# angelvillar96/STLPose

Measured on AMD Instinct MI355X. Metric: images/sec/GPU HRNet-W32 384x288 train step; PCKh@0.5 parity, higher is better.
Workload: dtype f16/bf16; 1 GPU; HRNet-W32 384x288 bs=32/GPU train step (fwd+MSE+bwd+Adam), random-init weights; global_batch=32, parallelism=dp1

## Files before the change

stlpose_amd/csrc/common.cuh:

```cuda
#pragma once
#include <hip/hip_runtime.h>
#include <stdint.h>
#include <stdio.h>
#include <initializer_list>
#include <tuple>
#include <type_traits>
#include <utility>
#include "../../include/stlpose_hip.h"
#include "../../include/stlpose_hip_math.h"

typedef __attribute__((ext_vector_type(4))) float f32x4;
typedef __attribute__((ext_vector_type(8))) __bf16 bf16x8;
typedef __attribute__((ext_vector_type(8))) _Float16 f16x8;
typedef __attribute__((ext_vector_type(4))) short s16x4;
struct f32s { float v; };
typedef _Float16 f16;

struct alignas(16) V16 {
    uint32_t w[4];
};

int stl_set_error(const char* fmt, ...);
void stl_note_kernel(const char* name, bool specific);
#define STL_CHECK(cond, ...)                 \
// ... 283 lines not shown
    } else {
#pragma unroll
        for (int k = 0; k < STL_NSHARD; ++k) {
            r.rs[2 * k] = s.rstats[(size_t)k * 2 * C + c];
            r.rs[2 * k + 1] = s.rstats[(size_t)k * 2 * C + C + c];
        }
    }
}
__device__ __forceinline__ void src_raw_finish(const stl_src& s, const SrcRaw& r, float& ca, float& cb, float& cc) {
#pragma clang fp contract(off)
    if (s.mode == STL_SRC_PLAIN) {
        ca = 1.f, cb = 0.f, cc = 0.f;
        return;
    }
    float mean, rstd;
    bn_raw_finish(s, r, mean, rstd);
    if (s.mode == STL_SRC_BN || s.mode == STL_SRC_BNADD) {
        ca = r.g * rstd;
        cb = fmaf(-mean, ca, r.b);
        cc = 0.f;
    } else {
        double r1 = 0.0, r2 = 0.0;
#pragma unroll
        for (int k = 0; k < STL_NSHARD; ++k) r1 += r.rs[2 * k], r2 += r.rs[2 * k + 1];
        const float c1 = (float)(r1 * (double)s.inv_count);
        const float c2 = (float)(r2 * (double)s.inv_count);
        const float al = r.g * rstd;
        ca = al;
        cb = -al * rstd * c2;
        cc = al * fmaf(mean * rstd, c2, -c1);
    }
}

__device__ __forceinline__ float row16_sum(float v) {
    v += __int_as_float(__builtin_amdgcn_update_dpp(0, __float_as_int(v), 0xB1, 0xf, 0xf, true));
    v += __int_as_float(__builtin_amdgcn_update_dpp(0, __float_as_int(v), 0x4E, 0xf, 0xf, true));
    v += __int_as_float(__builtin_amdgcn_update_dpp(0, __float_as_int(v), 0x141, 0xf, 0xf, true));
    v += __int_as_float(__builtin_amdgcn_update_dpp(0, __float_as_int(v), 0x140, 0xf, 0xf, true));
    return v;
}

__device__ __forceinline__ float wave_sum(float v) {
#pragma unroll
    for (int o = 32; o > 0; o >>= 1) v += __shfl_xor(v, o);
    return v;
}
__device__ __forceinline__ double wave_sum_d(double v) {
#pragma unroll
    for (int o = 32; o > 0; o >>= 1) v += __shfl_xor(v, o);
    return v;
}

__device__ __forceinline__ bool better(float v, int i, float bv, int bi) {
    const bool vn = v != v, bn = bv != bv;
    if (vn != bn) return vn;
    if (vn) return i < bi;
    return v > bv || (v == bv && i < bi);
}
__device__ __forceinline__ void argmax_take(float v, int i, float& bv, int& bi) {
    if (bi == 0x7fffffff || better(v, i, bv, bi)) bv = v, bi = i;
}
__device__ __forceinline__ void block_argmax_reduce(float& bv, int& bi, float* sv, int* si) {
    for (int o = 32; o > 0; o >>= 1) {
        const float ov = __shfl_xor(bv, o);
        const int oi = __shfl_xor(bi, o);
        if (oi != 0x7fffffff && (bi == 0x7fffffff || better(ov, oi, bv, bi))) bv = ov, bi = oi;
// ... 41 lines not shown
```

stlpose_amd/csrc/conv1x1.inc:

```
template <typename T, int G, bool Q, int OCC, typename TY = T, int EO = -1, bool ZM = false>
__global__ __launch_bounds__(512, OCC) void conv1x1_kernel(const ConvK k) {
    extern __shared__ __attribute__((aligned(16))) char smem[];
    constexpr int NTHR = 512, WM = 4, MT = 4, NTW = 2, BCO = 64, TPX = 256;
    constexpr int KV = ET<T>::KV, CK = ET<T>::CK;
    constexpr int PSG = G * 64 + 32;
    constexpr int VPP = 4 * G;
    constexpr int RPT = NTHR / VPP;
    constexpr int NVA = TPX / RPT;
    constexpr int NVB = BCO / RPT;
    constexpr int GK = G * CK;
    static_assert(NVB >= 1, "filter staging needs at least one vector per thread");
    const stl_conv& p = k.p;
    const int tid = threadIdx.x, lane = tid & 63, wave = tid >> 6, r16 = lane & 15, g = lane >> 4;
    const int wm = wave % WM, wn = wave / WM;
    const int bl = blockIdx.x >> 3;
    const int by = bl % k.ny, lx = bl / k.ny;
    const int n0 = by * BCO;
    const int xcd = blockIdx.x & 7, nx = (gridDim.x >> 3) / k.ny;
    const int P = p.B * p.Ho * p.Wo;

    float* cs = reinterpret_cast<float*>(smem + k.off_cs);
    float* cm = reinterpret_cast<float*>(smem + k.off_cm);
    char* sA = smem + k.off_a;
    char* sB = smem + k.off_b;

    for (int c = tid; c < k.cipad; c += NTHR) {
        float a = 0.f, b = 0.f, cc = 0.f;
        if (c < p.Ci) src_consts(p.src, c, p.Ci, a, b, cc);
        cs[c] = a, cs[k.cipad + c] = b, cs[2 * k.cipad + c] = cc;
    }
    if (p.mask_y) {
        for (int c = tid; c < BCO; c += NTHR) {
            float a = 0.f, b = 0.f, mu = 0.f, rs = 0.f;
            if (n0 + c < p.Co) {
                bn_mean_rstd(p.mask_bn, n0 + c, p.Co, mu, rs);
                bn_affine(p.mask_bn.gamma[n0 + c], p.mask_bn.beta[n0 + c], mu, rs, a, b);
            }
            cm[c] = a, cm[BCO + c] = b, cm[2 * BCO + c] = mu, cm[3 * BCO + c] = rs;
        }
    }

    const int a_part = tid % VPP, a_row = tid / VPP;
    V16 ra[NVA], rq[Q ? NVA : 1], rb[NVB];

    auto issue = [&](int P0, int k0, bool en) {
        const int ch = k0 + a_part * KV;
        const bool chok = en && ch < p.Ci;
#pragma unroll
        for (int i = 0; i < NVA; ++i) {
            const int pix = P0 + a_row + i * RPT;
            const size_t off = (chok && pix < P) ? (size_t)pix * p.Ci + ch : 0;
            ra[i] = ldg16((const char*)p.src.x + off * sizeof(T));
            if (Q) rq[i] = ldg16((const char*)p.src.y + off * sizeof(T));
        }
        if (!k.wres) {
#pragma unroll
            for (int i = 0; i < NVB; ++i) {
                const int n = n0 + a_row + i * RPT;
                const size_t off = (chok && n < p.Co) ? (size_t)n * p.Ci + ch : 0;
                rb[i] = ldg16((const char*)p.w + off * sizeof(T));
            }
        }
    };
    const float relu_lo = p.src.relu ? 0.f : -INFINITY;
    auto write_lds = [&](int P0, int k0) {
        const int ch = k0 + a_part * KV;
        const bool chok = ch < p.Ci;
        const int chc = chok ? ch : 0;
#pragma unroll
        for (int i = 0; i < NVA; ++i) {
            const bool ok = chok && (P0 + a_row + i * RPT) < P;
            V16 val = ra[i];
            if constexpr (ZM) {
                val = xform_bnadd<T>(val, rq[i], cs + chc, cs + k.cipad + chc, relu_lo);
                if (ok && by == 0 && p.src_out) stg16((char*)p.src_out + ((size_t)(P0 + a_row + i * RPT) * p.Ci + ch) * sizeof(T), val);
            } else if (Q)
                val = xform_bnbwd<T, TY>(val, rq[i], cs + chc, cs + k.cipad + chc, cs + 2 * k.cipad + chc);
            else if (p.src.mode != STL_SRC_PLAIN)
                val = xform_bn<T>(val, cs + chc, cs + k.cipad + chc, relu_lo);
            mask16(val, ok);
            *reinterpret_cast<V16*>(sA + (a_row + i * RPT) * PSG + a_part * 16) = val;
        }
        if (!k.wres) {
#pragma unroll
            for (int i = 0; i < NVB; ++i) {
                V16 val = rb[i];
                mask16(val, chok && (n0 + a_row + i * RPT) < p.Co);
                *reinterpret_cast<V16*>(sB + (a_row + i * RPT) * PSG + a_part * 16) = val;
            }
        }
    };

    if (k.wres) {
        const bool chok = a_part * KV < p.Ci;
#pragma unroll
        for (int i = 0; i < NVB; ++i) {
            const int n = n0 + a_row + i * RPT;
            const size_t off = (chok && n < p.Co) ? (size_t)n * p.Ci + a_part * KV : 0;
            rb[i] = ldg16((const char*)p.w + off * sizeof(T));
        }
    }

    f2v s0[NTW][2], s1[NTW][2];
#pragma unroll
    for (int ni = 0; ni < NTW; ++ni)
#pragma unroll
        for (int h = 0; h < 2; ++h) s0[ni][h] = f2v{0.f, 0.f}, s1[ni][h] = f2v{0.f, 0.f};
    f32x4 acc[MT][NTW];
#pragma unroll
    for (int mi = 0; mi < MT; ++mi)
#pragma unroll
        for (int ni = 0; ni < NTW; ++ni) acc[mi][ni] = f32x4{0.f, 0.f, 0.f, 0.f};

    int xoff[MT];
#pragma unroll
    for (int mi = 0; mi < MT; ++mi) xoff[mi] = ((wm * MT + mi) * 16 + r16) * PSG + g * 16;
    const int woff = (wn * NTW * 16 + r16) * PSG + g * 16;

    const int T8 = (k.npt + 7) >> 3;
    int it = lx, t = xcd * T8 + it, ch0 = 0;
    bool have = (it < T8) && (t < k.npt);
    issue(t * TPX, 0, have);
    if (k.wres) {
        const bool chok = a_part * KV < p.Ci;
#pragma unroll
        for (int i = 0; i < NVB; ++i) {
            V16 val = rb[i];
            mask16(val, chok && (n0 + a_row + i * RPT) < p.Co);
            *reinterpret_cast<V16*>(sB + (a_row + i * RPT) * PSG + a_part * 16) = val;
        }
    }
    __syncthreads();

    while (have) {
        const int P0 = t * TPX;
        write_lds(P0, ch0 * GK);
        __syncthreads();
        const bool last_chunk = (ch0 + 1 == k.nchunks);
        int itn = it, tn = t, chn = ch0 + 1;
        bool have_n = true;
        if (last_chunk) {
            itn = it + nx, tn = xcd * T8 + itn, chn = 0;
            have_n = (itn < T8) && (tn < k.npt);
        }
        issue(tn * TPX, chn * GK, have_n);
#pragma unroll
        for (int sub = 0; sub < G; ++sub) {
            V16 wf[NTW], xf[MT];
#pragma unroll
            for (int ni = 0; ni < NTW; ++ni) wf[ni] = *reinterpret_cast<const V16*>(sB + woff + ni * 16 * PSG + sub * 64);
#pragma unroll
            for (int mi = 0; mi < MT; ++mi) xf[mi] = *reinterpret_cast<const V16*>(sA + xoff[mi] + sub * 64);
#pragma unroll
            for (int mi = 0; mi < MT; ++mi)
#pragma unroll
// ... 114 lines not shown
```

stlpose_amd/csrc/conv_core.hip:

```cpp
#include <stdlib.h>
#include <algorithm>
#include <cstring>
#include <type_traits>
#include "common.cuh"

#ifndef STL_DT
#define STL_DT 2
#endif
#define STL_HAS_F32 (STL_DT == 0 || STL_DT == 2)
#define STL_HAS_BF16 (STL_DT == 1 || STL_DT == 2)
#define STL_HAS_F16 (STL_DT == 3 || STL_DT == 2)
#define STL_HAS_F32S (STL_DT == 4 || STL_DT == 2)

struct ConvK {
    stl_conv p;
    int tiles_c, npt;
    int HR, HC, HP;
    int PI, pad, seff;
    int nchunks, wres;
    int cipad;
    int off_cs, off_cm, off_a, off_b, off_red;
    int sz_a, sz_b;
    int TH, TW;
    int dbg;
// ... 48 lines not shown

#ifndef STL_PIN_TAPS
#define STL_PIN_TAPS 1
#endif
#include "conv_common.inc"

template <typename T, int KS, int WM, int WN, int MT, int NTW, int NVA, bool Q, bool PE, int OCC, int WR, bool ZM = false, typename TY = T, bool DB = false, int EO = -1>
__global__ __launch_bounds__(64 * WM * WN, OCC) void conv_core_kernel(const ConvK k) {
    extern __shared__ __attribute__((aligned(16))) char smem[];
    constexpr int NTHR = 64 * WM * WN;
    constexpr int KV = ET<T>::KV, CK = ET<T>::CK, TAPS = KS * KS;
    static_assert(!ZM || (Q && KS == 3), "block-end source: 3x3, two tensors on load");
    static_assert(!DB || (!ZM && WR == 0 && KS == 3), "double-buffered image: 3x3, plain / BN / BNBWD sources, filters staged per chunk");
    constexpr int BCO = WN * NTW * 16;
    constexpr int ROWB = TAPS * 64 + 32;
    constexpr int NVB = (BCO * TAPS * 4 + NTHR - 1) / NTHR;
    const stl_conv& p = k.p;
    const int tid = threadIdx.x, lane = tid & 63, wave = tid >> 6, r16 = lane & 15, g = lane >> 4;
    const int wm = wave % WM, wn = wave / WM;
    const int bl = blockIdx.x >> 3;
    const int lx = __builtin_amdgcn_readfirstlane(bl / k.ny), by = bl - lx * k.ny;
    const int n0 = by * BCO;
    const bool wres = WR < 0 ? (k.wres != 0) : (WR == 1);

    STAMP(0);
#ifdef STL_STAMPS
    if (k.dbg && blockIdx.x == 0 && blockIdx.y == 0 && threadIdx.x == 0) g_stamps[12] = __builtin_amdgcn_s_memtime();
#endif
    float* cs = reinterpret_cast<float*>(smem + k.off_cs);
    float* cm = reinterpret_cast<float*>(smem + k.off_cm);
    char* sA = smem + k.off_a;
    char* sB = smem + k.off_b;

    for (int c = tid; c < k.cipad; c += NTHR) {
        float a = 0.f, b = 0.f, cc = 0.f;
        if (c < p.Ci) src_consts(p.src, c, p.Ci, a, b, cc);
        cs[c] = a, cs[k.cipad + c] = b, cs[2 * k.cipad + c] = cc;
    }
    if (!PE && EpiOps<EO>::my(p)) {
        for (int c = tid - (NTHR - 64); c >= 0 && c < BCO; c += 64) {
            float a = 0.f, b = 0.f, mu = 0.f, rs = 0.f;
            if (n0 + c < p.Co) {
                bn_mean_rstd(p.mask_bn, n0 + c, p.Co, mu, rs);
                bn_affine(p.mask_bn.gamma[n0 + c], p.mask_bn.beta[n0 + c], mu, rs, a, b);
            }
            cm[c] = a, cm[BCO + c] = b, cm[2 * BCO + c] = mu, cm[3 * BCO + c] = rs;
        }
    }
    STAMP(1);
    int a_rc[NVA];
#pragma unroll
    for (int i = 0; i < NVA; ++i) {
        const int v = tid + i * NTHR;
        if (v < k.HP * 4) {
            const int hp = v >> 2, hr = fdiv(hp, k.r_HC);
            a_rc[i] = (hr << 16) | (hp - hr * k.HC);
        } else {
            a_rc[i] = -1;
        }
    }
    const int a_part = tid & 3;
    uint32_t a_int = 0;
    if constexpr (ZM) {
#pragma unroll
        for (int i = 0; i < NVA; ++i)
            if (a_rc[i] >= 0) {
                const int hr = a_rc[i] >> 16, hc = a_rc[i] & 0xffff;
                if (hr >= 1 && hr <= k.TH && hc >= 1 && hc <= k.TW && by == 0 && p.src_out) a_int |= 1u << i;
            }
    }
    int b_g[NVB], b_l[NVB];
#pragma unroll
    for (int i = 0; i < NVB; ++i) {
        const int v = tid + i * NTHR;
        b_g[i] = -1, b_l[i] = 0;
        if (v < BCO * TAPS * 4) {
            const int n = v / (TAPS * 4), r = v - n * (TAPS * 4), tap = r >> 2, part = r & 3;
            b_l[i] = n * ROWB + tap * 64 + part * 16;
            if (n0 + n < p.Co) b_g[i] = ((n0 + n) * TAPS + tap) * p.Ci + part * KV;
        }
    }
    const int tilepx = k.TH * k.TW;
    int xoff[MT];
    int e_yx[MT];
#pragma unroll
    for (int mi = 0; mi < MT; ++mi) {
        int m = (wm * MT + mi) * 16 + r16;
        e_yx[mi] = -1;
        if (m < tilepx) {
            const int ty = fdiv(m, k.r_TW);
            e_yx[mi] = (ty << 16) | (m - ty * k.TW);
        } else {
            m = 0;
        }
        const int ty = fdiv(m, k.r_TW), tx = m - ty * k.TW;
        xoff[mi] = ((ty * k.seff) * k.HC + tx * k.seff) * PSA + g * 16;
    }
    const int woff = (wn * NTW * 16 + r16) * ROWB + g * 16;

    STAMP(2);
    V16 ra[NVA], rq[Q ? NVA : 1], rb[NVB];
    int a_go[NVA];
    int st_t, st_ch;
    bool st_have;

    auto tile_terms = [&](int t, int& y0, int& cb, int& b0) __attribute__((always_inline)) {
        const int tr = sdiv(t, k.m_tc), tc = t - tr * k.tiles_c;
        const int vrs = tr * k.TH * k.seff;
        cb = tc * k.TW * k.seff - k.pad;
        b0 = sdiv(vrs, k.m_PI), y0 = vrs - b0 * k.PI - k.pad;
    };
    auto slot_go = [&](int rc, int y0, int cb, int b0) __attribute__((always_inline)) -> int {
// ... 34 lines not shown
        }
    };
    const float relu_lo = p.src.relu ? 0.f : -INFINITY;
    auto write_lds = [&](const int* go, int k0) __attribute__((always_inline)) {
        const int ch = k0 + a_part * KV;
#pragma unroll
        for (int i = 0; i < NVA; ++i) {
            if (a_rc[i] < 0) continue;
            const bool ok = go[i] >= 0 && ch < p.Ci;
            const int chc = ok ? ch : 0;
            V16 val = ra[i];
            if constexpr (ZM) {
                val = xform_bnadd<T>(val, rq[i], cs + chc, cs + k.cipad + chc, relu_lo);
                if (ok && ((a_int >> i) & 1u)) stg16((char*)p.src_out + (size_t)(go[i] + k0) * sizeof(T), val);
            } else if (Q)
                val = xform_bnbwd<T, TY>(val, rq[i], cs + chc, cs + k.cipad + chc, cs + 2 * k.cipad + chc);
            else if (p.src.mode != STL_SRC_PLAIN)
                val = xform_bn<T>(val, cs + chc, cs + k.cipad + chc, relu_lo);
            mask16(val, ok);
            const int v = tid + i * NTHR;
            *reinterpret_cast<V16*>(sA + (v >> 2) * PSA + (v & 3) * 16) = val;
        }
        if (!wres) {
#pragma unroll
            for (int i = 0; i < NVB; ++i) {
                const bool ok = b_g[i] >= 0 && (k0 + ((tid + i * NTHR) & 3) * KV) < p.Ci;
                V16 val = rb[i];
                mask16(val, ok);
                if (tid + i * NTHR < BCO * TAPS * 4) *reinterpret_cast<V16*>(sB + b_l[i]) = val;
            }
        }
    };

    if (wres) {
#pragma unroll
        for (int i = 0; i < NVB; ++i) {
            const bool ok = b_g[i] >= 0 && (((tid + i * NTHR) & 3) * KV) < p.Ci;
            rb[i] = ldg16((const char*)p.w + (size_t)(ok ? b_g[i] : 0) * sizeof(T));
        }
    }

    f2v s0[NTW][2], s1[NTW][2];
#pragma unroll
    for (int ni = 0; ni < NTW; ++ni)
#pragma unroll
        for (int h = 0; h < 2; ++h) s0[ni][h] = f2v{0.f, 0.f}, s1[ni][h] = f2v{0.f, 0.f};

    const int xcd = blockIdx.x & 7, nx = __builtin_amdgcn_readfirstlane((gridDim.x >> 3) / k.ny);
    const int T8 = (k.npt + 7) >> 3;
    const int vpitch = p.Ho + 1;

    int it_n = lx, t_n = xcd * T8 + lx, ch_n = 0;
    bool have_n = (it_n < T8) && (t_n < k.npt);
    auto prefetch = [&]() __attribute__((always_inline)) {
        if (have_n && ch_n == 0) tile_setup(t_n, a_go);
        st_t = t_n, st_ch = ch_n, st_have = have_n;
        issue(a_go, ch_n * CK, have_n);
        if (++ch_n == k.nchunks) {
            ch_n = 0, it_n += nx, t_n = xcd * T8 + it_n;
            have_n = have_n && (it_n < T8) && (t_n < k.npt);
        }
    };
    STAMP(3);
    if constexpr (!DB) {
        prefetch();
        if (wres) {
#pragma unroll
            for (int i = 0; i < NVB; ++i) {
                const bool ok = b_g[i] >= 0 && (((tid + i * NTHR) & 3) * KV) < p.Ci;
                V16 val = rb[i];
                mask16(val, ok);
                if (tid + i * NTHR < BCO * TAPS * 4) *reinterpret_cast<V16*>(sB + b_l[i]) = val;
            }
        }
        __syncthreads();
    }
    STAMP(4);

    f32x4 acc[MT][NTW];
#pragma unroll
    for (int mi = 0; mi < MT; ++mi)
#pragma unroll
        for (int ni = 0; ni < NTW; ++ni) acc[mi][ni] = f32x4{0.f, 0.f, 0.f, 0.f};

    constexpr bool EPRE = (OCC <= 1 && WM == 4 && WN == 2 && NTW == 2) && Q && !PE && !ZM && sizeof(T) == 2;
    constexpr bool EBURST = !EPRE && (EO == 1 || EO == 2) && !PE && sizeof(T) == 2;
    auto out_pixel = [&](int vr0, int c0, int mi, bool& pok) __attribute__((always_inline)) -> size_t {
        const int eb0 = sdiv(vr0, k.m_vp), ey0 = vr0 - eb0 * vpitch;
        int eyx = e_yx[mi];
        if constexpr (DB) {
            const int m = (wm * MT + mi) * 16 + r16, ty_ = fdiv(m, k.r_TW);
            eyx = m < tilepx ? ((ty_ << 16) | (m - ty_ * k.TW)) : -1;
        }
        const int ty = eyx >> 16, tx = eyx & 0xffff;
        const int oy0 = ey0 + ty, c = c0 + tx;
        const int wr_ = fdiv(oy0, k.r_vp);
        const int oy = mad24_vsv(wr_, -vpitch, oy0), b = eb0 + wr_;
        pok = (eyx >= 0) & (b < p.B) & (oy < p.Ho) & (c < p.Wo);
        const int e = mulu24_vs(madu24_vsv(madu24_vsv(b, p.Ho, oy), p.Wo, c), p.Co);
        return pok ? (size_t)(uint32_t)e : 0;
    };
    auto epi_fetch = [&](int vr0, int c0, bool* pokv, size_t* pixv, EpiRaw<NTW>* er) __attribute__((always_inline)) {
#pragma unroll
        for (int mi = 0; mi < MT; ++mi) {
            pixv[mi] = out_pixel(vr0, c0, mi, pokv[mi]);
            epilogue_fetch<T, NTW, true, EO>(p, pokv[mi], pixv[mi], n0, wn * NTW * 16, g, er[mi]);
        }
    };

    if constexpr (DB) {
        constexpr int NSLOT = NVA + NVB;
        prefetch();
        int cu_t = st_t, cu_ch = st_ch;
        bool cu_have = st_have;
        __syncthreads();
        write_lds(a_go, st_ch * CK);
        prefetch();
        __syncthreads();
        int img = 0;
        [[maybe_unused]] int dbg_it = 0;
        while (cu_have) {
            STAMP2(4 * dbg_it);
            const int t = cu_t, ch0 = cu_ch;
            const int tr = sdiv(t, k.m_tc), tc = t - tr * k.tiles_c;
            const int vr0 = tr * k.TH, c0 = tc * k.TW;
            const bool last_chunk = (ch0 + 1 == k.nchunks);
            bool pokv[EPRE ? MT : 1];
            size_t pixv[EPRE ? MT : 1];
            EpiRaw<NTW> er[EPRE ? MT : 1];
            const int k0w = st_ch * CK, k0n = ch_n * CK;
            const bool en_n = have_n, nt = have_n && ch_n == 0;
            int y0n = 0, cbn = 0, b0n = 0;
            if (nt) tile_terms(t_n, y0n, cbn, b0n);
            constexpr bool KREG = !Q || EO == 0 || EO == 1 || EO == 2;
            constexpr int NPK = sizeof(T) == 2 ? 4 : 2;
            f2v kca[NPK], kcb[NPK], kcc[Q ? NPK : 1];
            if constexpr (KREG) {
                const int ch = k0w + a_part * KV;
#pragma unroll
                for (int i = 0; i < NPK; ++i) {
                    kca[i] = reinterpret_cast<const f2v*>(cs + ch)[i];
                    kcb[i] = reinterpret_cast<const f2v*>(cs + k.cipad + ch)[i];
                    if (Q) kcc[i] = reinterpret_cast<const f2v*>(cs + 2 * k.cipad + ch)[i];
                }
            }
// ... 621 lines not shown
```

stlpose_amd/csrc/elementwise.hip:

```cpp
#include "common.cuh"

namespace {

template <typename T>
__device__ __forceinline__ void load8(const void* base, size_t elem, float* f) {
    if constexpr (sizeof(T) == 2) {
        unpack<T>(ldg16((const char*)base + elem * 2), f);
    } else {
        unpack<float>(ldg16((const char*)base + elem * 4), f);
        unpack<float>(ldg16((const char*)base + elem * 4 + 16), f + 4);
    }
}
template <typename T>
__device__ __forceinline__ void store8(void* base, size_t elem, const float* f) {
    if constexpr (sizeof(T) == 2) {
        stg16((char*)base + elem * 2, pack<T>(f));
    } else {
        stg16((char*)base + elem * 4, pack<float>(f));
        stg16((char*)base + elem * 4 + 16, pack<float>(f + 4));
    }
}

template <int NS>
__device__ __forceinline__ void flush_sets(float (*acc)[8], float* red, int C, int VPC, double* const* dst,
                                           const int* which, int nsets) {
    const int tid = threadIdx.x, nthr = blockDim.x;
    __syncthreads();
#pragma unroll
    for (int s = 0; s < NS; ++s)
#pragma unroll
        for (int j = 0; j < 8; ++j) red[(tid * NS + s) * 8 + j] = acc[s][j];
    __syncthreads();
    for (int e = tid; e < nsets * C; e += nthr) {
        const int s = e / C, c = e - s * C, cg = c >> 3, j = c & 7;
        float sum = 0.f;
        for (int q = cg; q < nthr; q += VPC) sum += red[(q * NS + s) * 8 + j];
        atomicAdd(dst[s] + (size_t)(blockIdx.x & (STL_NSHARD - 1)) * 2 * C + which[s] * C + c, (double)sum);
    }
}

template <typename T>
__global__ __launch_bounds__(256) void fuse_fwd_kernel(const stl_fuse p) {
    extern __shared__ __attribute__((aligned(16))) char smem[];
    float* cs = reinterpret_cast<float*>(smem);
    const int C = p.C, VPC = C >> 3;
    for (int e = threadIdx.x; e < p.nterms * C; e += blockDim.x) {
        const int t = e / C, c = e - t * C;
        float a, b, cc;
        src_consts(p.t[t].src, c, C, a, b, cc);
        cs[(t * 2) * C + c] = a, cs[(t * 2 + 1) * C + c] = b;
    }
    __syncthreads();
    const uint32_t total = (uint32_t)p.B * p.H * p.W * VPC;
    bool flat = true;
    for (int t = 0; t < p.nterms; ++t) flat = flat && p.t[t].shift == 0;
    for (uint32_t v = blockIdx.x * blockDim.x + threadIdx.x; v < total; v += gridDim.x * blockDim.x) {
        const uint32_t pi = v / (uint32_t)VPC;
        const int c0 = (int)(v - pi * VPC) * 8;
        int x = 0, y = 0, b = 0;
        if (!flat) {
            const uint32_t by = pi / (uint32_t)p.W;
            x = (int)(pi - by * p.W);
            b = (int)(by / (uint32_t)p.H);
            y = (int)(by - (uint32_t)b * p.H);
        }
        float s[8];
#pragma unroll
        for (int j = 0; j < 8; ++j) s[j] = 0.f;
        for (int t = 0; t < p.nterms; ++t) {
            const stl_term& tm = p.t[t];
            const int hs = p.H >> tm.shift, ws = p.W >> tm.shift;
            const size_t off = flat ? (size_t)v * 8 : (((size_t)b * hs + (y >> tm.shift)) * ws + (x >> tm.shift)) * C + c0;
            float f[8];
            load8<T>(tm.src.x, off, f);
            if (tm.src.mode == STL_SRC_BN) {
#pragma unroll
                for (int j = 0; j < 8; ++j) {
                    float u = fmaf(cs[(t * 2) * C + c0 + j], f[j], cs[(t * 2 + 1) * C + c0 + j]);
                    f[j] = tm.src.relu ? max_lo<T>(u, 0.f) : u;
                }
            }
#pragma unroll
            for (int j = 0; j < 8; ++j) s[j] += f[j];
        }
        if (p.relu) {
#pragma unroll
            for (int j = 0; j < 8; ++j) s[j] = max_lo<T>(s[j], 0.f);
        }
        store8<T>(p.out, (size_t)v * 8, s);
    }
}

template <typename T>
__global__ __launch_bounds__(256) void fuse_flat_big_kernel(const stl_fuse p) {
    extern __shared__ __attribute__((aligned(16))) char smem[];
    float* cs = reinterpret_cast<float*>(smem);
    const int C = p.C, VPC = C >> 3;
    for (int e = threadIdx.x; e < p.nterms * C; e += blockDim.x) {
        const int t = e / C, c = e - t * C;
        float a, b, cc;
        src_consts(p.t[t].src, c, C, a, b, cc);
        cs[(t * 2) * C + c] = a, cs[(t * 2 + 1) * C + c] = b;
    }
    __syncthreads();
    const uint32_t total = (uint32_t)p.B * p.H * p.W * VPC;
    const uint32_t nthr = gridDim.x * blockDim.x;
    const uint32_t v0 = blockIdx.x * blockDim.x + threadIdx.x;
    const int c0 = (int)(v0 % (uint32_t)VPC) * 8;
    float ca[2][8], cb[2][8];
#pragma unroll
    for (int t = 0; t < 2; ++t)
#pragma unroll
        for (int j = 0; j < 8; ++j) {
            ca[t][j] = t < p.nterms ? cs[(t * 2) * C + c0 + j] : 0.f;
            cb[t][j] = t < p.nterms ? cs[(t * 2 + 1) * C + c0 + j] : 0.f;
        }
    const bool two = p.nterms == 2;
    const bool bn0 = p.t[0].src.mode == STL_SRC_BN, bn1 = two && p.t[1].src.mode == STL_SRC_BN;
    const bool r0 = p.t[0].src.relu, r1 = two && p.t[1].src.relu;
    const void* x0 = p.t[0].src.x;
    const void* x1 = two ? p.t[1].src.x : p.t[0].src.x;
    auto term = [&](float* f, const float* a, const float* b, bool bn, bool relu) __attribute__((always_inline)) {
// ... 23 lines not shown
            term(fb, ca[1], cb[1], bn1, r1);
#pragma unroll
            for (int j = 0; j < 8; ++j) s[j] += fb[j];
        }
        if (p.relu) {
#pragma unroll
            for (int j = 0; j < 8; ++j) s[j] = max_lo<T>(s[j], 0.f);
        }
        store8<T>(p.out, (size_t)v * 8, s);
        if (hw) {
            term(ga, ca[0], cb[0], bn0, r0);
#pragma unroll
            for (int j = 0; j < 8; ++j) s[j] = 0.f + ga[j];
            if (two) {
                term(gb, ca[1], cb[1], bn1, r1);
#pragma unroll
                for (int j = 0; j < 8; ++j) s[j] += gb[j];
            }
            if (p.relu) {
#pragma unroll
                for (int j = 0; j < 8; ++j) s[j] = max_lo<T>(s[j], 0.f);
            }
            store8<T>(p.out, (size_t)w * 8, s);
        }
    }
}

template <typename T, typename TY = T>
__global__ __launch_bounds__(256, sizeof(T) == 4 ? 2 : 4) void fuse_bwd_kernel(const stl_fuse_bwd p) {
    extern __shared__ __attribute__((aligned(16))) char smem[];
    const int C = p.C, VPC = C >> 3;
    float* mu = reinterpret_cast<float*>(smem);
    float* red = mu + (size_t)(p.nbn > 0 ? p.nbn : 1) * 2 * C;
    for (int e = threadIdx.x; e < p.nbn * C; e += blockDim.x) {
        const int t = e / C, c = e - t * C;
        float m, r;
        bn_mean_rstd(p.bn[t], c, C, m, r);
        mu[(t * 2) * C + c] = m, mu[(t * 2 + 1) * C + c] = r;
    }
    __syncthreads();
    float acc[5][8];
#pragma unroll
    for (int s = 0; s < 5; ++s)
#pragma unroll
        for (int j = 0; j < 8; ++j) acc[s][j] = 0.f;
    const size_t total = (size_t)p.B * p.H * p.W * VPC;
    const int cg = threadIdx.x % VPC, c0 = cg * 8;
    const void* dzp[4];
    const void* yp[4];
#pragma unroll
    for (int k = 0; k < 4; ++k) dzp[k] = k < p.ngrads ? p.dz[k] : p.dz[0];
#pragma unroll
    for (int t = 0; t < 4; ++t) yp[t] = t < p.nbn ? p.bn[t].x : p.dz[0];
    const void* zp = p.relu ? p.z : p.dz[0];
    for (size_t v = (size_t)blockIdx.x * blockDim.x + threadIdx.x; v < total; v += (size_t)gridDim.x * blockDim.x) {
        const size_t off = v * 8;
        float d[8], e1[8], e2[8], e3[8], z[8], y[4][8];
        load8<T>(dzp[0], off, d);
        load8<T>(dzp[1], off, e1);
        load8<T>(dzp[2], off, e2);
        load8<T>(dzp[3], off, e3);
        load8<TY>(zp, off, z);
#pragma unroll
        for (int t = 0; t < 4; ++t) load8<TY>(yp[t], off, y[t]);
        if (p.ngrads > 1) {
#pragma unroll
            for (int j = 0; j < 8; ++j) d[j] += e1[j];
        }
        if (p.ngrads > 2) {
#pragma unroll
            for (int j = 0; j < 8; ++j) d[j] += e2[j];
        }
        if (p.ngrads > 3) {
#pragma unroll
            for (int j = 0; j < 8; ++j) d[j] += e3[j];
        }
        if (p.relu) {
#pragma unroll
            for (int j = 0; j < 8; ++j) d[j] = z[j] > 0.f ? d[j] : 0.f;
        }
#pragma unroll
        for (int j = 0; j < 8; ++j) d[j] = round_to<T>(d[j]);
        store8<T>(p.du, off, d);
        if (p.nbn > 0) {
#pragma unroll
            for (int j = 0; j < 8; ++j) acc[0][j] += d[j];
#pragma unroll
            for (int t = 0; t < 4; ++t) {
                if (t < p.nbn) {
#pragma unroll
                    for (int j = 0; j < 8; ++j)
                        acc[1 + t][j] += d[j] * (y[t][j] - mu[(t * 2) * C + c0 + j]) * mu[(t * 2 + 1) * C + c0 + j];
                }
            }
        }
    }
    if (p.nbn > 0) {
        double* dst[5];
        int which[5];
#pragma unroll
        for (int t = 0; t < 4; ++t) {
            if (t < p.nbn) {
                dst[0] = p.rstats[t], which[0] = 0;
                dst[1] = p.rstats[t], which[1] = 1;
                float two[2][8];
#pragma unroll
                for (int j = 0; j < 8; ++j) two[0][j] = acc[0][j], two[1][j] = acc[1 + t][j];
                flush_sets<2>(two, red, C, VPC, dst, which, 2);
            }
        }
    }
}

template <typename T, typename TY, int SHIFT>
__global__ __launch_bounds__(256) void upsample_bwd_kernel(const stl_upbwd p) {
    extern __shared__ __attribute__((aligned(16))) char smem[];
    const int C = p.C, VPC = C >> 3;
    float* mu = reinterpret_cast<float*>(smem);
    float* red = mu + 2 * C;
    for (int c = threadIdx.x; c < C; c += blockDim.x) {
        float m, r;
        bn_mean_rstd(p.bn, c, C, m, r);
        mu[c] = m, mu[C + c] = r;
    }
    __syncthreads();
    float acc[2][8];
#pragma unroll
    for (int s = 0; s < 2; ++s)
#pragma unroll
        for (int j = 0; j < 8; ++j) acc[s][j] = 0.f;
    constexpr int F = 1 << SHIFT;
    const uint32_t Wh = (uint32_t)p.W << SHIFT, Hh = (uint32_t)p.H << SHIFT;
    const uint32_t total = (uint32_t)p.B * p.H * p.W * VPC;
    const int cg = threadIdx.x % VPC, c0 = cg * 8;
    for (uint32_t v = blockIdx.x * blockDim.x + threadIdx.x; v < total; v += gridDim.x * blockDim.x) {
        const uint32_t pi = v / (uint32_t)VPC;
        const uint32_t by = pi / (uint32_t)p.W, x = pi - by * p.W;
        const uint32_t b = by / (uint32_t)p.H, y = by - b * p.H;
        float yv[8];
        load8<TY>(p.bn.x, (size_t)pi * C + c0, yv);
        float s[8];
#pragma unroll
        for (int j = 0; j < 8; ++j) s[j] = 0.f;
        const size_t row0 = ((size_t)(b * Hh + y * F) * Wh + x * F) * C + c0;
#pragma unroll(SHIFT == 1 ? 2 : 1)
        for (int dy = 0; dy < F; ++dy) {
            float d[F][8];
#pragma unroll
            for (int dx = 0; dx < F; ++dx) load8<T>(p.du, row0 + ((size_t)dy * Wh + dx) * C, d[dx]);
#pragma unroll
            for (int dx = 0; dx < F; ++dx)
#pragma unroll
                for (int j = 0; j < 8; ++j) s[j] += d[dx][j];
        }
#pragma unroll
        for (int j = 0; j < 8; ++j) s[j] = round_to<T>(s[j]);
        store8<T>(p.dt, (size_t)pi * C + c0, s);
#pragma unroll
        for (int j = 0; j < 8; ++j) {
            acc[0][j] += s[j];
            acc[1][j] += s[j] * (yv[j] - mu[c0 + j]) * mu[C + c0 + j];
        }
    }
    double* dst[2] = {p.rstats, p.rstats};
    int which[2] = {0, 1};
    flush_sets<2>(acc, red, C, VPC, dst, which, 2);
}

template <typename T>
__global__ __launch_bounds__(256) void patch_kernel(const float* img, void* out, int B, int H, int W, int Ho, int Wo,
                                                    int stride, const float* mean3, const float* std3) {
    const size_t total = (size_t)B * Ho * Wo * 4;
    float mean[3] = {0.f, 0.f, 0.f}, istd[3] = {1.f, 1.f, 1.f};
    if (mean3) {
#pragma unroll
        for (int c = 0; c < 3; ++c) mean[c] = mean3[c], istd[c] = 1.f / std3[c];
    }
    for (size_t v = (size_t)blockIdx.x * 256 + threadIdx.x; v < total; v += (size_t)gridDim.x * 256) {
        const size_t pi = v >> 2;
        const int part = (int)(v & 3);
        const int ox = (int)(pi % Wo);
        const size_t by = pi / Wo;
        const int oy = (int)(by % Ho), b = (int)(by / Ho);
        float f[8];
#pragma unroll
        for (int j = 0; j < 8; ++j) {
            const int kk = part * 8 + j;
            float val = 0.f;
            if (kk < 27) {
                const int tap = kk / 3, c = kk - tap * 3;
                const int iy = oy * stride + tap / 3 - 1, ix = ox * stride + tap % 3 - 1;
                if (iy >= 0 && iy < H && ix >= 0 && ix < W) {
                    val = img[(((size_t)b * 3 + c) * H + iy) * W + ix];
                    if (mean3) val = (val - mean[c]) / std3[c];
                }
            }
// ... 1259 lines not shown
```

Before: 2474 images/sec.

## Overlap per-channel BN constant setup with first-tile global loads across kernels

Splits the per-channel batch-norm constant computation into a raw-load phase and a finish phase so the first tile's activation and weight loads are issued before the constants are reduced and written to shared memory. This applies to the conv1x1 and generic conv kernels, the multi-term add kernel, the BN backward kernel and the upsample backward kernel, hiding prologue latency that was serialized before the main loop. It also swaps one filter-offset computation for a 24-bit multiply-add. The cost is extra live registers for the prefetched data, which may reduce occupancy, plus more complex first-iteration code paths.

```diff
diff --git a/stlpose_amd/csrc/common.cuh b/stlpose_amd/csrc/common.cuh
--- a/stlpose_amd/csrc/common.cuh
+++ b/stlpose_amd/csrc/common.cuh
@@ -339,6 +339,62 @@
     }
 }
 
+template <int NTHR, int BCO, bool TAIL = true>
+struct ConvConsts {
+    SrcRaw raw;
+    int nitem, it_c;
+    bool it_src, it_ok;
+    __device__ __forceinline__ void load(const stl_src& src, const stl_src& mbn, int Ci, int Co, int cipad, int n0, bool need_cm, float* cs, float* cm) {
+        const int tid = threadIdx.x;
+        nitem = cipad + (need_cm ? BCO : 0);
+        it_src = tid < cipad;
+        it_c = it_src ? tid : n0 + (tid - cipad);
+        it_ok = it_src ? (tid < Ci) : (tid < nitem && it_c < Co);
+        if (TAIL && __builtin_expect(nitem > NTHR, 0))
+        for (int item = tid + NTHR; item < nitem; item += NTHR) {
+            if (item < cipad) {
+                float a = 0.f, b = 0.f, cc = 0.f;
+                if (item < Ci) src_consts(src, item, Ci, a, b, cc);
+                cs[item] = a, cs[cipad + item] = b, cs[2 * cipad + item] = cc;
+            } else {
+                const int c = item - cipad;
+                float a = 0.f, b = 0.f, mu = 0.f, rs = 0.f;
+                if (n0 + c < Co) {
+                    bn_mean_rstd(mbn, n0 + c, Co, mu, rs);
+                    bn_affine(mbn.gamma[n0 + c], mbn.beta[n0 + c], mu, rs, a, b);
+                }
+                cm[c] = a, cm[BCO + c] = b, cm[2 * BCO + c] = mu, cm[3 * BCO + c] = rs;
+            }
+        }
+        if (it_ok) {
+            if (it_src) {
+                src_raw_load(src, it_c, Ci, raw);
+            } else {
+                bn_raw_load(mbn, it_c, Co, raw);
+                raw.b = mbn.beta[it_c];
+            }
+        }
+    }
+    __device__ __forceinline__ void finish(const stl_src& src, const stl_src& mbn, int Ci, int Co, int cipad, int n0, float* cs, float* cm) const {
+        const int tid = threadIdx.x;
+        if (tid < nitem) {
+            if (it_src) {
+                float a = 0.f, b = 0.f, cc = 0.f;
+                if (it_ok) src_raw_finish(src, raw, a, b, cc);
+                cs[tid] = a, cs[cipad + tid] = b, cs[2 * cipad + tid] = cc;
+            } else {
+                float a = 0.f, b = 0.f, mu = 0.f, rs = 0.f;
+                if (it_ok) {
+                    bn_raw_finish(mbn, raw, mu, rs);
+                    bn_affine(raw.g, raw.b, mu, rs, a, b);
+                }
+                const int c = tid - cipad;
+                cm[c] = a, cm[BCO + c] = b, cm[2 * BCO + c] = mu, cm[3 * BCO + c] = rs;
+            }
+        }
+    }
+};
+
 __device__ __forceinline__ float row16_sum(float v) {
     v += __int_as_float(__builtin_amdgcn_update_dpp(0, __float_as_int(v), 0xB1, 0xf, 0xf, true));
     v += __int_as_float(__builtin_amdgcn_update_dpp(0, __float_as_int(v), 0x4E, 0xf, 0xf, true));
diff --git a/stlpose_amd/csrc/conv1x1.inc b/stlpose_amd/csrc/conv1x1.inc
--- a/stlpose_amd/csrc/conv1x1.inc
+++ b/stlpose_amd/csrc/conv1x1.inc
@@ -24,21 +24,8 @@
     char* sA = smem + k.off_a;
     char* sB = smem + k.off_b;
 
-    for (int c = tid; c < k.cipad; c += NTHR) {
-        float a = 0.f, b = 0.f, cc = 0.f;
-        if (c < p.Ci) src_consts(p.src, c, p.Ci, a, b, cc);
-        cs[c] = a, cs[k.cipad + c] = b, cs[2 * k.cipad + c] = cc;
-    }
-    if (p.mask_y) {
-        for (int c = tid; c < BCO; c += NTHR) {
-            float a = 0.f, b = 0.f, mu = 0.f, rs = 0.f;
-            if (n0 + c < p.Co) {
-                bn_mean_rstd(p.mask_bn, n0 + c, p.Co, mu, rs);
-                bn_affine(p.mask_bn.gamma[n0 + c], p.mask_bn.beta[n0 + c], mu, rs, a, b);
-            }
-            cm[c] = a, cm[BCO + c] = b, cm[2 * BCO + c] = mu, cm[3 * BCO + c] = rs;
-        }
-    }
+    ConvConsts<NTHR, BCO> kc;
+    kc.load(p.src, p.mask_bn, p.Ci, p.Co, k.cipad, n0, p.mask_y != nullptr, cs, cm);
 
     const int a_part = tid % VPP, a_row = tid / VPP;
     V16 ra[NVA], rq[Q ? NVA : 1], rb[NVB];
@@ -91,6 +78,26 @@
         }
     };
 
+    f2v s0[NTW][2], s1[NTW][2];
+#pragma unroll
+    for (int ni = 0; ni < NTW; ++ni)
+#pragma unroll
+        for (int h = 0; h < 2; ++h) s0[ni][h] = f2v{0.f, 0.f}, s1[ni][h] = f2v{0.f, 0.f};
+    f32x4 acc[MT][NTW];
+#pragma unroll
+    for (int mi = 0; mi < MT; ++mi)
+#pragma unroll
+        for (int ni = 0; ni < NTW; ++ni) acc[mi][ni] = f32x4{0.f, 0.f, 0.f, 0.f};
+
+    int xoff[MT];
+#pragma unroll
+    for (int mi = 0; mi < MT; ++mi) xoff[mi] = ((wm * MT + mi) * 16 + r16) * PSG + g * 16;
+    const int woff = (wn * NTW * 16 + r16) * PSG + g * 16;
+
+    const int T8 = (k.npt + 7) >> 3;
+    int it = lx, t = xcd * T8 + it, ch0 = 0;
+    bool have = (it < T8) && (t < k.npt);
+    issue(t * TPX, 0, have);
     if (k.wres) {
         const bool chok = a_part * KV < p.Ci;
 #pragma unroll
@@ -100,27 +107,7 @@
             rb[i] = ldg16((const char*)p.w + off * sizeof(T));
         }
     }
-
-    f2v s0[NTW][2], s1[NTW][2];
-#pragma unroll
-    for (int ni = 0; ni < NTW; ++ni)
-#pragma unroll
-        for (int h = 0; h < 2; ++h) s0[ni][h] = f2v{0.f, 0.f}, s1[ni][h] = f2v{0.f, 0.f};
-    f32x4 acc[MT][NTW];
-#pragma unroll
-    for (int mi = 0; mi < MT; ++mi)
-#pragma unroll
-        for (int ni = 0; ni < NTW; ++ni) acc[mi][ni] = f32x4{0.f, 0.f, 0.f, 0.f};
-
-    int xoff[MT];
-#pragma unroll
-    for (int mi = 0; mi < MT; ++mi) xoff[mi] = ((wm * MT + mi) * 16 + r16) * PSG + g * 16;
-    const int woff = (wn * NTW * 16 + r16) * PSG + g * 16;
-
-    const int T8 = (k.npt + 7) >> 3;
-    int it = lx, t = xcd * T8 + it, ch0 = 0;
-    bool have = (it < T8) && (t < k.npt);
-    issue(t * TPX, 0, have);
+    kc.finish(p.src, p.mask_bn, p.Ci, p.Co, k.cipad, n0, cs, cm);
     if (k.wres) {
         const bool chok = a_part * KV < p.Ci;
 #pragma unroll
diff --git a/stlpose_amd/csrc/conv_core.hip b/stlpose_amd/csrc/conv_core.hip
--- a/stlpose_amd/csrc/conv_core.hip
+++ b/stlpose_amd/csrc/conv_core.hip
@@ -104,21 +104,9 @@
     char* sA = smem + k.off_a;
     char* sB = smem + k.off_b;
 
-    for (int c = tid; c < k.cipad; c += NTHR) {
-        float a = 0.f, b = 0.f, cc = 0.f;
-        if (c < p.Ci) src_consts(p.src, c, p.Ci, a, b, cc);
-        cs[c] = a, cs[k.cipad + c] = b, cs[2 * k.cipad + c] = cc;
-    }
-    if (!PE && EpiOps<EO>::my(p)) {
-        for (int c = tid - (NTHR - 64); c >= 0 && c < BCO; c += 64) {
-            float a = 0.f, b = 0.f, mu = 0.f, rs = 0.f;
-            if (n0 + c < p.Co) {
-                bn_mean_rstd(p.mask_bn, n0 + c, p.Co, mu, rs);
-                bn_affine(p.mask_bn.gamma[n0 + c], p.mask_bn.beta[n0 + c], mu, rs, a, b);
-            }
-            cm[c] = a, cm[BCO + c] = b, cm[2 * BCO + c] = mu, cm[3 * BCO + c] = rs;
-        }
-    }
+    static_assert(WR != 1 || CK + BCO <= NTHR, "resident filters: one K chunk, never more constant items than threads");
+    ConvConsts<NTHR, BCO, WR != 1> kc;
+    kc.load(p.src, p.mask_bn, p.Ci, p.Co, k.cipad, n0, !PE && EpiOps<EO>::my(p), cs, cm);
     STAMP(1);
     int a_rc[NVA];
 #pragma unroll
@@ -149,7 +137,7 @@
         if (v < BCO * TAPS * 4) {
             const int n = v / (TAPS * 4), r = v - n * (TAPS * 4), tap = r >> 2, part = r & 3;
             b_l[i] = n * ROWB + tap * 64 + part * 16;
-            if (n0 + n < p.Co) b_g[i] = ((n0 + n) * TAPS + tap) * p.Ci + part * KV;
+            if (n0 + n < p.Co) b_g[i] = madu24_vsv(madu24_vsv(n0 + n, TAPS, tap), p.Ci, part * KV);
         }
     }
     const int tilepx = k.TH * k.TW;
@@ -250,14 +238,6 @@
         }
     };
 
-    if (wres) {
-#pragma unroll
-        for (int i = 0; i < NVB; ++i) {
-            const bool ok = b_g[i] >= 0 && (((tid + i * NTHR) & 3) * KV) < p.Ci;
-            rb[i] = ldg16((const char*)p.w + (size_t)(ok ? b_g[i] : 0) * sizeof(T));
-        }
-    }
-
     f2v s0[NTW][2], s1[NTW][2];
 #pragma unroll
     for (int ni = 0; ni < NTW; ++ni)
@@ -279,9 +259,17 @@
             have_n = have_n && (it_n < T8) && (t_n < k.npt);
         }
     };
+    prefetch();
+    if (wres) {
+#pragma unroll
+        for (int i = 0; i < NVB; ++i) {
+            const bool ok = b_g[i] >= 0 && (((tid + i * NTHR) & 3) * KV) < p.Ci;
+            rb[i] = ldg16((const char*)p.w + (size_t)(ok ? b_g[i] : 0) * sizeof(T));
+        }
+    }
     STAMP(3);
+    kc.finish(p.src, p.mask_bn, p.Ci, p.Co, k.cipad, n0, cs, cm);
     if constexpr (!DB) {
-        prefetch();
         if (wres) {
 #pragma unroll
             for (int i = 0; i < NVB; ++i) {
@@ -328,7 +316,6 @@
 
     if constexpr (DB) {
         constexpr int NSLOT = NVA + NVB;
-        prefetch();
         int cu_t = st_t, cu_ch = st_ch;
         bool cu_have = st_have;
         __syncthreads();
diff --git a/stlpose_amd/csrc/elementwise.hip b/stlpose_amd/csrc/elementwise.hip
--- a/stlpose_amd/csrc/elementwise.hip
+++ b/stlpose_amd/csrc/elementwise.hip
@@ -12,6 +12,28 @@
     }
 }
 template <typename T>
+struct Raw8 {
+    V16 v[sizeof(T) == 2 ? 1 : 2];
+};
+template <typename T>
+__device__ __forceinline__ void raw8_load(const void* base, size_t elem, Raw8<T>& r) {
+    if constexpr (sizeof(T) == 2) {
+        r.v[0] = ldg16((const char*)base + elem * 2);
+    } else {
+        r.v[0] = ldg16((const char*)base + elem * 4);
+        r.v[1] = ldg16((const char*)base + elem * 4 + 16);
+    }
+}
+template <typename T>
+__device__ __forceinline__ void raw8_unpack(const Raw8<T>& r, float* f) {
+    if constexpr (sizeof(T) == 2) {
+        unpack<T>(r.v[0], f);
+    } else {
+        unpack<float>(r.v[0], f);
+        unpack<float>(r.v[1], f + 4);
+    }
+}
+template <typename T>
 __device__ __forceinline__ void store8(void* base, size_t elem, const float* f) {
     if constexpr (sizeof(T) == 2) {
         stg16((char*)base + elem * 2, pack<T>(f));
@@ -44,50 +66,100 @@
     extern __shared__ __attribute__((aligned(16))) char smem[];
     float* cs = reinterpret_cast<float*>(smem);
     const int C = p.C, VPC = C >> 3;
-    for (int e = threadIdx.x; e < p.nterms * C; e += blockDim.x) {
-        const int t = e / C, c = e - t * C;
-        float a, b, cc;
-        src_consts(p.t[t].src, c, C, a, b, cc);
-        cs[(t * 2) * C + c] = a, cs[(t * 2 + 1) * C + c] = b;
-    }
-    __syncthreads();
+    const int nitem = p.nterms * C;
+    const int e0 = threadIdx.x, t0 = e0 / C, ch0 = e0 - t0 * C;
+    SrcRaw raw;
+    if (e0 < nitem) src_raw_load(p.t[t0].src, ch0, C, raw);
     const uint32_t total = (uint32_t)p.B * p.H * p.W * VPC;
     bool flat = true;
     for (int t = 0; t < p.nterms; ++t) flat = flat && p.t[t].shift == 0;
-    for (uint32_t v = blockIdx.x * blockDim.x + threadIdx.x; v < total; v += gridDim.x * blockDim.x) {
+    auto term_off = [&](const stl_term& tm, uint32_t v, int c0, int x, int y, int b) __attribute__((always_inline)) -> size_t {
+        const int hs = p.H >> tm.shift, ws = p.W >> tm.shift;
+        return flat ? (size_t)v * 8 : (((size_t)b * hs + (y >> tm.shift)) * ws + (x >> tm.shift)) * C + c0;
+    };
+    auto coords = [&](uint32_t v, int& c0, int& x, int& y, int& b) __attribute__((always_inline)) {
         const uint32_t pi = v / (uint32_t)VPC;
-        const int c0 = (int)(v - pi * VPC) * 8;
-        int x = 0, y = 0, b = 0;
+        c0 = (int)(v - pi * VPC) * 8;
+        x = 0, y = 0, b = 0;
         if (!flat) {
             const uint32_t by = pi / (uint32_t)p.W;
             x = (int)(pi - by * p.W);
             b = (int)(by / (uint32_t)p.H);
             y = (int)(by - (uint32_t)b * p.H);
         }
+    };
+    auto term_apply = [&](const stl_term& tm, int t, int c0, float* f) __attribute__((always_inline)) {
+        if (tm.src.mode == STL_SRC_BN) {
+#pragma unroll
+            for (int j = 0; j < 8; ++j) {
+                float u = fmaf(cs[(t * 2) * C + c0 + j], f[j], cs[(t * 2 + 1) * C + c0 + j]);
+                f[j] = tm.src.relu ? max_lo<T>(u, 0.f) : u;
+            }
+        }
+    };
+    auto finish = [&](uint32_t v, float* s) __attribute__((always_inline)) {
+        if (p.relu) {
+#pragma unroll
+            for (int j = 0; j < 8; ++j) s[j] = max_lo<T>(s[j], 0.f);
+        }
+        store8<T>(p.out, (size_t)v * 8, s);
+    };
+    constexpr bool PRE = sizeof(T) == 2;
+    const uint32_t stride = gridDim.x * blockDim.x, v0 = blockIdx.x * blockDim.x + threadIdx.x;
+    const bool have0 = PRE && v0 < total;
+    Raw8<T> r0[PRE ? 4 : 1];
+    int c00 = 0, x0, y0, b0;
+    if constexpr (PRE) {
+        coords(have0 ? v0 : 0, c00, x0, y0, b0);
+#pragma unroll
+        for (int t = 0; t < 4; ++t) {
+            const stl_term& tm = p.t[t < p.nterms ? t : 0];
+            raw8_load<T>(tm.src.x, term_off(tm, have0 ? v0 : 0, c00, x0, y0, b0), r0[t]);
+        }
+    }
+    if (e0 < nitem) {
+        float a, b, cc;
+        src_raw_finish(p.t[t0].src, raw, a, b, cc);
+        cs[(t0 * 2) * C + ch0] = a, cs[(t0 * 2 + 1) * C + ch0] = b;
+    }
+    for (int e = e0 + blockDim.x; e < nitem; e += blockDim.x) {
+        const int t = e / C, c = e - t * C;
+        float a, b, cc;
+        src_consts(p.t[t].src, c, C, a, b, cc);
+        cs[(t * 2) * C + c] = a, cs[(t * 2 + 1) * C + c] = b;
+    }
+    __syncthreads();
+    if (have0) {
+        float s[8];
+#pragma unroll
+        for (int j = 0; j < 8; ++j) s[j] = 0.f;
+#pragma unroll
+        for (int t = 0; t < 4; ++t) {
+            if (t < p.nterms) {
+                float f[8];
+                raw8_unpack<T>(r0[PRE ? t : 0], f);
+                term_apply(p.t[t], t, c00, f);
+#pragma unroll
+                for (int j = 0; j < 8; ++j) s[j] += f[j];
+            }
+        }
+        finish(v0, s);
+    }
+    for (uint32_t v = PRE ? v0 + stride : v0; v < total; v += stride) {
+        int c0, x, y, b;
+        coords(v, c0, x, y, b);
         float s[8];
 #pragma unroll
         for (int j = 0; j < 8; ++j) s[j] = 0.f;
         for (int t = 0; t < p.nterms; ++t) {
             const stl_term& tm = p.t[t];
-            const int hs = p.H >> tm.shift, ws = p.W >> tm.shift;
-            const size_t off = flat ? (size_t)v * 8 : (((size_t)b * hs + (y >> tm.shift)) * ws + (x >> tm.shift)) * C + c0;
             float f[8];
-            load8<T>(tm.src.x, off, f);
-            if (tm.src.mode == STL_SRC_BN) {
-#pragma unroll
-                for (int j = 0; j < 8; ++j) {
-                    float u = fmaf(cs[(t * 2) * C + c0 + j], f[j], cs[(t * 2 + 1) * C + c0 + j]);
-                    f[j] = tm.src.relu ? max_lo<T>(u, 0.f) : u;
-                }
-            }
+            load8<T>(tm.src.x, term_off(tm, v, c0, x, y, b), f);
+            term_apply(tm, t, c0, f);
 #pragma unroll
             for (int j = 0; j < 8; ++j) s[j] += f[j];
         }
-        if (p.relu) {
-#pragma unroll
-            for (int j = 0; j < 8; ++j) s[j] = max_lo<T>(s[j], 0.f);
-        }
-        store8<T>(p.out, (size_t)v * 8, s);
+        finish(v, s);
     }
 }
 
@@ -177,18 +249,10 @@
     const int C = p.C, VPC = C >> 3;
     float* mu = reinterpret_cast<float*>(smem);
     float* red = mu + (size_t)(p.nbn > 0 ? p.nbn : 1) * 2 * C;
-    for (int e = threadIdx.x; e < p.nbn * C; e += blockDim.x) {
-        const int t = e / C, c = e - t * C;
-        float m, r;
-        bn_mean_rstd(p.bn[t], c, C, m, r);
-        mu[(t * 2) * C + c] = m, mu[(t * 2 + 1) * C + c] = r;
-    }
-    __syncthreads();
-    float acc[5][8];
-#pragma unroll
-    for (int s = 0; s < 5; ++s)
-#pragma unroll
-        for (int j = 0; j < 8; ++j) acc[s][j] = 0.f;
+    const int nitem = p.nbn * C;
+    const int e0 = threadIdx.x, t0 = e0 / C, ch0 = e0 - t0 * C;
+    SrcRaw raw;
+    if (e0 < nitem) bn_raw_load(p.bn[t0], ch0, C, raw);
     const size_t total = (size_t)p.B * p.H * p.W * VPC;
     const int cg = threadIdx.x % VPC, c0 = cg * 8;
     const void* dzp[4];
@@ -198,16 +262,48 @@
 #pragma unroll
     for (int t = 0; t < 4; ++t) yp[t] = t < p.nbn ? p.bn[t].x : p.dz[0];
     const void* zp = p.relu ? p.z : p.dz[0];
-    for (size_t v = (size_t)blockIdx.x * blockDim.x + threadIdx.x; v < total; v += (size_t)gridDim.x * blockDim.x) {
+    struct Elem {
+        Raw8<T> d[4];
+        Raw8<TY> z, y[4];
+    };
+    auto fetch = [&](size_t off, Elem& r) __attribute__((always_inline)) {
+#pragma unroll
+        for (int k = 0; k < 4; ++k) raw8_load<T>(dzp[k], off, r.d[k]);
+        raw8_load<TY>(zp, off, r.z);
+#pragma unroll
+        for (int t = 0; t < 4; ++t) raw8_load<TY>(yp[t], off, r.y[t]);
+    };
+    const size_t v0 = (size_t)blockIdx.x * blockDim.x + threadIdx.x, stride = (size_t)gridDim.x * blockDim.x;
+    Elem r;
+    fetch(v0 < total ? v0 * 8 : 0, r);
+    if (e0 < nitem) {
+        float m, rs;
+        bn_raw_finish(p.bn[t0], raw, m, rs);
+        mu[(t0 * 2) * C + ch0] = m, mu[(t0 * 2 + 1) * C + ch0] = rs;
+    }
+    for (int e = e0 + blockDim.x; e < nitem; e += blockDim.x) {
+        const int t = e / C, c = e - t * C;
+        float m, rs;
+        bn_mean_rstd(p.bn[t], c, C, m, rs);
+        mu[(t * 2) * C + c] = m, mu[(t * 2 + 1) * C + c] = rs;
+    }
+    __syncthreads();
+    float acc[5][8];
+#pragma unroll
+    for (int s = 0; s < 5; ++s)
+#pragma unroll
+        for (int j = 0; j < 8; ++j) acc[s][j] = 0.f;
+    for (size_t v = v0; v < total; v += stride) {
         const size_t off = v * 8;
+        if (v != v0) fetch(off, r);
         float d[8], e1[8], e2[8], e3[8], z[8], y[4][8];
-        load8<T>(dzp[0], off, d);
-        load8<T>(dzp[1], off, e1);
-        load8<T>(dzp[2], off, e2);
-        load8<T>(dzp[3], off, e3);
-        load8<TY>(zp, off, z);
-#pragma unroll
-        for (int t = 0; t < 4; ++t) load8<TY>(yp[t], off, y[t]);
+        raw8_unpack<T>(r.d[0], d);
+        raw8_unpack<T>(r.d[1], e1);
+        raw8_unpack<T>(r.d[2], e2);
+        raw8_unpack<T>(r.d[3], e3);
+        raw8_unpack<TY>(r.z, z);
+#pragma unroll
+        for (int t = 0; t < 4; ++t) raw8_unpack<TY>(r.y[t], y[t]);
         if (p.ngrads > 1) {
 #pragma unroll
             for (int j = 0; j < 8; ++j) d[j] += e1[j];
@@ -263,41 +359,85 @@
     const int C = p.C, VPC = C >> 3;
     float* mu = reinterpret_cast<float*>(smem);
     float* red = mu + 2 * C;
-    for (int c = threadIdx.x; c < C; c += blockDim.x) {
-        float m, r;
-        bn_mean_rstd(p.bn, c, C, m, r);
-        mu[c] = m, mu[C + c] = r;
-    }
-    __syncthreads();
-    float acc[2][8];
-#pragma unroll
-    for (int s = 0; s < 2; ++s)
-#pragma unroll
-        for (int j = 0; j < 8; ++j) acc[s][j] = 0.f;
+    const int e0 = threadIdx.x;
+    SrcRaw raw;
+    if (sizeof(T) == 2 && e0 < C) bn_raw_load(p.bn, e0, C, raw);
     constexpr int F = 1 << SHIFT;
     const uint32_t Wh = (uint32_t)p.W << SHIFT, Hh = (uint32_t)p.H << SHIFT;
     const uint32_t total = (uint32_t)p.B * p.H * p.W * VPC;
     const int cg = threadIdx.x % VPC, c0 = cg * 8;
-    for (uint32_t v = blockIdx.x * blockDim.x + threadIdx.x; v < total; v += gridDim.x * blockDim.x) {
-        const uint32_t pi = v / (uint32_t)VPC;
+    constexpr int RG = SHIFT == 1 ? 2 : 1;
+    constexpr bool PRE_Y = sizeof(T) == 2, PRE_D = PRE_Y;
+    auto origin = [&](uint32_t v, uint32_t& pi, size_t& row0) __attribute__((always_inline)) {
+        pi = v / (uint32_t)VPC;
         const uint32_t by = pi / (uint32_t)p.W, x = pi - by * p.W;
         const uint32_t b = by / (uint32_t)p.H, y = by - b * p.H;
+        row0 = ((size_t)(b * Hh + y * F) * Wh + x * F) * C + c0;
+    };
+    auto rows = [&](size_t row0, int dy, Raw8<T> (*rd)[F]) __attribute__((always_inline)) {
+#pragma unroll
+        for (int q = 0; q < RG; ++q)
+#pragma unroll
+            for (int dx = 0; dx < F; ++dx) raw8_load<T>(p.du, row0 + ((size_t)(dy + q) * Wh + dx) * C, rd[q][dx]);
+    };
+    const uint32_t v0 = blockIdx.x * blockDim.x + threadIdx.x, stride = gridDim.x * blockDim.x;
+    const bool have0 = PRE_Y && v0 < total;
+    Raw8<TY> ry0;
+    Raw8<T> rd0[RG][F];
+    if constexpr (PRE_Y) {
+        uint32_t pi;
+        size_t row0;
+        origin(have0 ? v0 : 0, pi, row0);
+        raw8_load<TY>(p.bn.x, (size_t)pi * C + c0, ry0);
+        if constexpr (PRE_D) rows(row0, 0, rd0);
+    }
+    if (PRE_Y && e0 < C) {
+        float m, rs;
+        bn_raw_finish(p.bn, raw, m, rs);
+        mu[e0] = m, mu[C + e0] = rs;
+    }
+    for (int c = PRE_Y ? e0 + blockDim.x : e0; c < C; c += blockDim.x) {
+        float m, rs;
+        bn_mean_rstd(p.bn, c, C, m, rs);
+        mu[c] = m, mu[C + c] = rs;
+    }
+    __syncthreads();
+    float acc[2][8];
+#pragma unroll
+    for (int s = 0; s < 2; ++s)
+#pragma unroll
+        for (int j = 0; j < 8; ++j) acc[s][j] = 0.f;
+    auto element = [&](uint32_t v, auto first_c) __attribute__((always_inline)) {
+        constexpr bool FIRST = decltype(first_c)::value;
+        uint32_t pi;
+        size_t row0;
+        origin(v, pi, row0);
+        Raw8<TY> ry;
+        if constexpr (FIRST) ry = ry0;
+        else raw8_load<TY>(p.bn.x, (size_t)pi * C + c0, ry);
         float yv[8];
-        load8<TY>(p.bn.x, (size_t)pi * C + c0, yv);
         float s[8];
 #pragma unroll
         for (int j = 0; j < 8; ++j) s[j] = 0.f;
-        const size_t row0 = ((size_t)(b * Hh + y * F) * Wh + x * F) * C + c0;
-#pragma unroll(SHIFT == 1 ? 2 : 1)
-        for (int dy = 0; dy < F; ++dy) {
-            float d[F][8];
-#pragma unroll
-            for (int dx = 0; dx < F; ++dx) load8<T>(p.du, row0 + ((size_t)dy * Wh + dx) * C, d[dx]);
-#pragma unroll
-            for (int dx = 0; dx < F; ++dx)
-#pragma unroll
-                for (int j = 0; j < 8; ++j) s[j] += d[dx][j];
-        }
+        auto add_rows = [&](const Raw8<T> (*rd)[F]) __attribute__((always_inline)) {
+#pragma unroll
+            for (int q = 0; q < RG; ++q)
+#pragma unroll
+                for (int dx = 0; dx < F; ++dx) {
+                    float d[8];
+                    raw8_unpack<T>(rd[q][dx], d);
+#pragma unroll
+                    for (int j = 0; j < 8; ++j) s[j] += d[j];
+                }
+        };
+        if constexpr (FIRST && PRE_D) add_rows(rd0);
+#pragma unroll 1
+        for (int dy = (FIRST && PRE_D) ? RG : 0; dy < F; dy += RG) {
+            Raw8<T> rd[RG][F];
+            rows(row0, dy, rd);
+            add_rows(rd);
+        }
+        raw8_unpack<TY>(ry, yv);
 #pragma unroll
         for (int j = 0; j < 8; ++j) s[j] = round_to<T>(s[j]);
         store8<T>(p.dt, (size_t)pi * C + c0, s);
@@ -306,7 +446,9 @@
             acc[0][j] += s[j];
             acc[1][j] += s[j] * (yv[j] - mu[c0 + j]) * mu[C + c0 + j];
         }
-    }
+    };
+    if (have0) element(v0, std::true_type{});
+    for (uint32_t v = PRE_Y ? v0 + stride : v0; v < total; v += stride) element(v, std::false_type{});
     double* dst[2] = {p.rstats, p.rstats};
     int which[2] = {0, 1};
     flush_sets<2>(acc, red, C, VPC, dst, which, 2);
```

New measurement: 2489 images/sec (median of 6 runs). No clear change (+0.6%).
